# kthohr/mcmc

Measured on AMD Instinct MI355X. Metric: leapfrog-steps/sec (chains*dims*steps/s), HMC d=128 correlated Gaussian, 65536 chains, higher is better.
Workload: dtype f64

## Files before the change

mcmc_amd/csrc/logistic_dense_m_impl.hpp:

```cpp
#pragma once
#include "logistic_lds_impl.hpp"

namespace mi {
namespace {

constexpr int dense_m_matrices(int algo) { return algo == LOGIT_MALA ? 3 : 2; }

template <int NTQ, int TARGET>
size_t dense_m_doubles(uint32_t d, uint64_t C, int algo)
{
    using G = LogitGeo<NTQ>;
    const size_t nbm = (d + 15) / 16, n_wg = (C + 31) / 32;
    return (size_t)dense_m_matrices(algo) * nbm * G::XBUF_PAD + (TARGET == LOGIT_TARGET_DENSE ? 0 : n_wg * 2 * 4 * G::NSQ * 64);
}

template <int NTQ, int ALGO, int TARGET>
int launch_dense_m(LogitParams& prm, const double* X_dev, const double* y_dev, void* workspace, void* mws, hipStream_t st)
{
    using G = LogitGeo<NTQ>;
    const size_t n_wg = (prm.C + 31) / 32;
    const uint32_t nbm = (prm.d + 15) / 16;
    const size_t img = (size_t)nbm * G::XBUF_PAD;
    double* xp = static_cast<double*>(workspace);
    prm.state = xp + (size_t)prm.NB * G::XBUF_PAD;
    double* m0 = static_cast<double*>(mws);
    prm.xexch = (TARGET == LOGIT_TARGET_DENSE) ? prm.state + n_wg * 8 * LOGIT_STATE_VECS * G::NSQ * 64 : m0 + (size_t)dense_m_matrices(ALGO) * img;
    prm.Xp = xp;
    hipLaunchKernelGGL((pack_logit_lds_kernel<NTQ, TARGET == LOGIT_TARGET_DENSE>), dim3(prm.NB), dim3(256), 0, st, X_dev, y_dev, prm.d, prm.n_rows, xp);
    auto pack = [&](const double* rm, double* dst) {
        hipLaunchKernelGGL((pack_logit_lds_kernel<NTQ, true>), dim3(nbm), dim3(256), 0, st, rm, nullptr, prm.d, prm.d, dst);
    };
    prm.Lp = m0; pack(prm.L_rm, m0);
    if (ALGO == LOGIT_MALA) {
        prm.Mp = m0 + img; pack(prm.M_rm, m0 + img);
        prm.Sip = m0 + 2 * img; pack(prm.Sinv_rm, m0 + 2 * img);
    } else {
        prm.Mip = m0 + img; pack(prm.Minv_rm, m0 + img);
    }
    auto kern = logit_lds_kernel<NTQ, ALGO, TARGET, false, false, true>;
    note_kernel("logit_lds_kernel<%d, %d, %d, false, false, true>", NTQ, ALGO, TARGET);
    hipError_t e = hipFuncSetAttribute(reinterpret_cast<const void*>(kern), hipFuncAttributeMaxDynamicSharedMemorySize, (int)G::LDS_BYTES);
    if (e != hipSuccess) return (int)e;
    hipLaunchKernelGGL(kern, dim3((unsigned)n_wg), dim3(512), G::LDS_BYTES, st, prm);
    return (int)hipGetLastError();
}

template <int ALGO>
int launch_dense_m_any(LogitParams& prm, const double* X_dev, const double* y_dev, void* workspace, void* mws, hipStream_t st, int target)
{
    if (target == LOGIT_TARGET_DENSE) {
        if (prm.d <= 192) return launch_dense_m<3, ALGO, LOGIT_TARGET_DENSE>(prm, X_dev, y_dev, workspace, mws, st);
        if (prm.d <= 256) return launch_dense_m<4, ALGO, LOGIT_TARGET_DENSE>(prm, X_dev, y_dev, workspace, mws, st);
        if (prm.d <= 384) return launch_dense_m<6, ALGO, LOGIT_TARGET_DENSE>(prm, X_dev, y_dev, workspace, mws, st);
        return launch_dense_m<8, ALGO, LOGIT_TARGET_DENSE>(prm, X_dev, y_dev, workspace, mws, st);
    }
    if (prm.d <= 64) return launch_dense_m<1, ALGO, LOGIT_TARGET_LOGISTIC>(prm, X_dev, y_dev, workspace, mws, st);
    if (prm.d <= 128) return launch_dense_m<2, ALGO, LOGIT_TARGET_LOGISTIC>(prm, X_dev, y_dev, workspace, mws, st);
    if (prm.d <= 256) return launch_dense_m<4, ALGO, LOGIT_TARGET_LOGISTIC>(prm, X_dev, y_dev, workspace, mws, st);
    return launch_dense_m<8, ALGO, LOGIT_TARGET_LOGISTIC>(prm, X_dev, y_dev, workspace, mws, st);
}

}
}
```

mcmc_amd/csrc/logistic_launch.hpp:

```cpp
#pragma once

#include <hip/hip_runtime.h>
#include <stddef.h>
#include <stdint.h>

namespace mi {

struct LogitParams {
    const double* Xp;
    uint32_t d, n_rows, NB;
    uint64_t C, chain0;
    double* theta;
    double* state;
    double* draws;
    uint64_t* n_accept;
    uint64_t seed;
    uint32_t n_burnin, n_keep, n_leap;
    uint32_t draw0;
    double eps, s2, rs, cons_term, log_det;
    uint32_t* nf_flag;
    const double* m_sqrt;
    const double* m_inv;
    const double* m;
    const double* s_inv;
    const int* btype;
    const double* lb;
    const double* ub;
    double* xexch;
    double* nuts_ws;
    double* nuts_sc;
    uint32_t* nuts_next;
    uint64_t* n_leap_out;
    uint64_t* n_exec_out;
    double* step_out;
    uint32_t* depth_trace;
    double* adapt_state;
    uint32_t n_adapt, max_depth;
    double delta, eps_bar0, gamma, t0, kappa;
    const double* Minv_rm;
    const double* L_rm;
    const double* M_rm;
    const double* Sinv_rm;
    const double* Mip;
    const double* Lp;
    const double* Mp;
    const double* Sip;
    uint32_t n_pieces, piece_len;
    uint32_t* piece_q;
    uint32_t* piece_tail;
    void* split_ws;
};

enum { LOGIT_MALA = 0, LOGIT_HMC = 1, LOGIT_RWMH = 2, LOGIT_NUTS = 3 };
enum { LOGIT_TARGET_LOGISTIC = 0, LOGIT_TARGET_DENSE = 1 };

size_t logit_lds_workspace_bytes(uint32_t d, uint32_t NB, uint64_t C, int target = LOGIT_TARGET_LOGISTIC, int algo = LOGIT_HMC);
uint64_t logit_lds_nuts_workgroups(uint32_t d, uint64_t C, int target);
size_t logit_lds_nuts_split_bytes(uint64_t C, uint32_t d);
size_t logit_lds_dense_m_bytes(uint32_t d, uint64_t C, int target, int algo);
int logit_lds_launch_dense_m(int algo, LogitParams prm, const double* X_dev, const double* y_dev, void* workspace, void* mws, hipStream_t st, int target);
size_t logit_lds_nuts_dense_m_bytes(uint32_t d, uint64_t C, int target);
uint64_t logit_lds_nuts_dense_m_workgroups(uint32_t d, uint64_t C, int target);
int logit_lds_launch_nuts_dense_m(LogitParams prm, const double* X_dev, const double* y_dev, void* workspace, void* mws, hipStream_t st, int target);
int logit_lds_launch_hmc_dense_m(LogitParams prm, const double* X_dev, const double* y_dev, void* workspace, void* mws, hipStream_t st, int target);
int logit_lds_launch_mala_dense_m(LogitParams prm, const double* X_dev, const double* y_dev, void* workspace, void* mws, hipStream_t st, int target);
int logit_lds_launch(int algo, LogitParams prm, const double* X_dev, const double* y_dev, void* workspace, hipStream_t st,
                     int target = LOGIT_TARGET_LOGISTIC);

}
```

mcmc_amd/csrc/logistic_lds.hpp:

```cpp
#pragma once

#include "hmc_dense.hpp"
#include "logistic_launch.hpp"
#include "nuts_lds.hpp"
#include "lds_box.hpp"

#ifndef MI_LOGIT_ABLATE
#define MI_LOGIT_ABLATE 0
#endif
#ifndef MI_LOGIT_BATCH
#define MI_LOGIT_BATCH 8
#endif

namespace mi {


constexpr int LOGIT_STATE_VECS = 3;

template <int NTQ>
struct LogitGeo {
    static constexpr int NSQ = 4 * NTQ;
    static constexpr int DQ = 16 * NTQ;
    static constexpr int DP = 64 * NTQ;
    static constexpr int RSP = 2 * DP + 34;
    static constexpr int XBUF = 8 * RSP;
    static constexpr int CHUNKS = (XBUF * 8 + 1023) / 1024;
    static constexpr int XBUF_PAD = CHUNKS * 128;
    static_assert(CHUNKS * 128 >= XBUF + 16, "no room for the labels");
    static constexpr int EXCH = 2 * (4 * 4 * 64 + 4 * 2 * 64);
    static constexpr size_t LDS_BYTES = (size_t)(2 * XBUF_PAD + EXCH) * sizeof(double);
    __host__ __device__ static constexpr int xaddr(int row, int dim) { return (row >> 1) * RSP + (row & 1) * (DP + 16) + dim; }
};

template <int NTQ>
inline size_t logit_lds_ws_doubles(uint32_t NB, uint64_t C, int target, int algo)
{
    using G = LogitGeo<NTQ>;
    const size_t n_wg = (C + 31) / 32;
    return (size_t)NB * G::XBUF_PAD + n_wg * 8 * LOGIT_STATE_VECS * G::NSQ * 64 + (target == LOGIT_TARGET_DENSE ? n_wg * 2 * 4 * G::NSQ * 64 : 0)
           + (algo == LOGIT_NUTS ? n_wg * 8 * (lds_nuts::vec_doubles_per_wave(G::NSQ) + lds_nuts::sc_doubles_per_wave()) + 32 : 0);
}
int logit_lds_launch_nuts(LogitParams prm, const double* X_dev, const double* y_dev, void* workspace, hipStream_t st, int target);

template <int NTQ, bool TRANSPOSED>
__global__ void pack_logit_lds_kernel(const double* __restrict__ X, const double* __restrict__ y, uint32_t d, uint32_t n_rows,
                                      double* Xp)
{
    using G = LogitGeo<NTQ>;
    const uint32_t b = blockIdx.x;
    double* img = Xp + (size_t)b * G::XBUF_PAD;
    for (int i = threadIdx.x; i < G::XBUF_PAD; i += blockDim.x) img[i] = 0.0;
    __syncthreads();
    for (int i = threadIdx.x; i < 16 * G::DP; i += blockDim.x) {
        const int r = i / G::DP, j = i % G::DP;
        const uint32_t row = 16 * b + r;
        if (row < n_rows && (uint32_t)j < d) img[G::xaddr(r, j)] = TRANSPOSED ? X[(size_t)j * d + row] : X[(size_t)row * d + j];
    }
    if (!TRANSPOSED && threadIdx.x < 16) {
        const uint32_t row = 16 * b + threadIdx.x;
        img[G::XBUF + threadIdx.x] = row < n_rows ? y[row] : 0.0;
    }
}

#ifndef MI_LOGIT_NUTS_W1
#define MI_LOGIT_NUTS_W1 2
#endif
template <int NTQ, int ALGO> constexpr int logit_waves_per_simd() { return (ALGO == LOGIT_NUTS && NTQ == 1) ? MI_LOGIT_NUTS_W1 : 2; }
template <int NTQ, int ALGO, int TARGET, bool DIAGM = false, bool BOUNDS = false, bool DENSEM = false>
__global__ MI_NO_DS_MERGE __launch_bounds__(512, (logit_waves_per_simd<NTQ, ALGO>())) void logit_lds_kernel(const LogitParams prm)
{
    static_assert(!BOUNDS || (DIAGM && (ALGO == LOGIT_HMC || ALGO == LOGIT_NUTS)), "bounds: hmc and nuts, with the mass tables");
    static_assert(!DENSEM || ((ALGO == LOGIT_HMC || ALGO == LOGIT_MALA || ALGO == LOGIT_NUTS) && !DIAGM && !BOUNDS), "a dense precond_mat: hmc, mala and nuts without bounds");
    using G = LogitGeo<NTQ>;
    constexpr int NSQ = G::NSQ, DQ = G::DQ, DP = G::DP, RSP = G::RSP;
    extern __shared__ double smem[];
    double* const Xs = smem;
    double* const part_all = smem + 2 * G::XBUF_PAD;
    double* const rt_all = part_all + 2 * 4 * 4 * 64;

    const int lane = threadIdx.x & 63;
    const int w = __builtin_amdgcn_readfirstlane((int)(threadIdx.x >> 6));
    const int g = w >> 2, q = w & 3;
    const int j4 = lane >> 4;
    const uint32_t d = prm.d;
    const uint64_t C = prm.C;
    const double eps = prm.eps;
    const uint32_t NB = prm.NB;
    constexpr uint32_t ablate = MI_LOGIT_ABLATE;
    const uint64_t t0_clk = (ablate & 1024u) ? clock64() : 0, t0_wall = (ablate & 1024u) ? wall_clock64() : 0;
    const uint64_t cl = ((uint64_t)blockIdx.x * 2 + g) * 16 + (lane & 15);
    const bool live = cl < C;
    const uint64_t chain = prm.chain0 + cl;
    double* const part = part_all + g * (4 * 4 * 64);
    double* const rt = rt_all + g * (4 * 2 * 64);
    double* const ws_wave = prm.state + ((size_t)blockIdx.x * 8 + w) * ((size_t)LOGIT_STATE_VECS * NSQ * 64) + lane;
    auto st = [&](int v, int s) -> double* {
        double* b = ws_wave + ((size_t)v * NSQ + (s & ~7)) * 64;
        asm volatile("" : "+v"(b));
        return b + (s & 7) * 64;
    };
    auto dim_of = [&](int s) -> uint32_t {
        uint32_t j = (uint32_t)j4;
        asm volatile("" : "+v"(j));
        return (uint32_t)(q * DQ + 4 * s) + j;
    };

    [[maybe_unused]] auto mass_at = [&](const double* tab, int s) __attribute__((always_inline)) -> double {
        uint32_t off = (uint32_t)j4 * 8u;
        asm volatile("" : "+v"(off));
        return *reinterpret_cast<const double*>(reinterpret_cast<const char*>(tab + (q * DQ + 4 * s)) + off);
    };

    const int eta_off = G::xaddr(lane & 15, q * DQ + j4);
    const int grad_off = (j4 >> 1) * RSP + (j4 & 1) * (DP + 16) + q * DQ + (lane & 15);

    const uint32_t xs_lds = (uint32_t)(uintptr_t)(__attribute__((address_space(3))) double*)Xs;
    auto issue_block = [&](uint32_t b, int buf) __attribute__((always_inline)) {
        const double* src = prm.Xp + (size_t)b * G::XBUF_PAD + lane * 2;
        const uint32_t dst = xs_lds + (uint32_t)buf * (uint32_t)(G::XBUF_PAD * sizeof(double));
#pragma unroll
        for (int c0 = 0; c0 < G::CHUNKS; c0 += 8) {
            const int c = c0 + w;
            if (c < G::CHUNKS) {
                uint32_t m0_saved;
                asm volatile("s_mov_b32 %0, m0\n\ts_mov_b32 m0, %2\n\ts_nop 0\n\tglobal_load_lds_dwordx4 %1, off\n\ts_mov_b32 m0, %0"
                             : "=&s"(m0_saved) : "v"(src + (size_t)c * 128), "s"(dst + (uint32_t)c * 1024u) : "memory");
            }
        }
    };
    const uint32_t lane16 = (uint32_t)lane * 16u;
    auto issue_piece_of = [&](const double* img, uint32_t b, int buf, int i) __attribute__((always_inline)) {
        const int c = i * 8 + w;
        if (c < G::CHUNKS) {
            const double* src = img + (size_t)b * G::XBUF_PAD + (size_t)c * 128;
            const uint32_t dst = xs_lds + (uint32_t)buf * (uint32_t)(G::XBUF_PAD * sizeof(double)) + (uint32_t)c * 1024u;
            uint32_t m0_saved;
            asm volatile("s_mov_b32 %0, m0\n\ts_mov_b32 m0, %2\n\ts_nop 0\n\tglobal_load_lds_dwordx4 %1, %3\n\ts_mov_b32 m0, %0"
                         : "=&s"(m0_saved) : "v"(lane16), "s"(dst), "s"(src) : "memory");
        }
    };
    const double* next_img = prm.Xp;
    auto img_of_next = [&](const double* img, bool last) __attribute__((always_inline)) -> const double* {
        if constexpr (DENSEM) return last ? next_img : img; else return prm.Xp;
    };
    constexpr int NP = (G::CHUNKS + 7) / 8, NP_E = (NTQ + 1) / 2;
    static_assert(NP_E + 1 + (NTQ + 1) / 2 >= NP, "piece schedule does not cover the block");
    auto wait_loads = [&]() __attribute__((always_inline)) { asm volatile("s_waitcnt vmcnt(0)" ::: "memory"); };

    auto exchange = [&](double (&v)[2]) __attribute__((always_inline)) {
        __syncthreads();
        part[(0 * 4 + q) * 64 + lane] = v[0];
        part[(1 * 4 + q) * 64 + lane] = v[1];
        __syncthreads();
#pragma unroll
        for (int k = 0; k < 2; ++k)
            v[k] = ((part[(k * 4 + 0) * 64 + lane] + part[(k * 4 + 1) * 64 + lane]) + part[(k * 4 + 2) * 64 + lane])
                   + part[(k * 4 + 3) * 64 + lane];
    };

    auto blk_sync = [&]() __attribute__((always_inline)) { if constexpr (!(ablate & 16u)) __syncthreads(); };
    uint64_t prof[11] = {0, 0, 0, 0, 0, 0, 0, 0, 0, 0, 0};
    auto stamp = [&]() __attribute__((always_inline)) -> uint64_t { if constexpr ((ablate & 2048u) != 0) return clock64(); else return 0; };
    auto lap = [&](uint64_t& tp, int i) __attribute__((always_inline)) {
        if constexpr ((ablate & 2048u) != 0) { const uint64_t t = clock64(); prof[i] += t - tp; tp = t; }
    };
    uint32_t xbuf_next = 0;
    auto xbuf_parity = [&]() __attribute__((always_inline)) -> uint32_t {
        if constexpr (ALGO == LOGIT_NUTS) return (uint32_t)__builtin_amdgcn_readfirstlane((int)xbuf_next); else return xbuf_next;
    };
    auto evaluate_logit = [&](const double (&x)[NSQ], double (&gout)[NSQ], double& lp) __attribute__((always_inline)) {
        double4_t gacc[NTQ];
        double llq = 0.0;
#pragma unroll
        for (int t = 0; t < NTQ; ++t) gacc[t] = double4_t{0.0, 0.0, 0.0, 0.0};
        uint64_t te = stamp();
        const uint32_t xbuf0 = xbuf_parity();
        __syncthreads();
        lap(te, 8);
#pragma unroll 1
        for (uint32_t b = 0; b < NB; ++b) {
            const double* xb = Xs + ((xbuf0 + b) & 1u) * G::XBUF_PAD;
            uint64_t tp = stamp();
            const bool prefetch = !(ablate & 8u);
            const uint32_t nblk = (b + 1 < NB) ? b + 1 : 0u;
            const int nbuf = (int)((xbuf0 + b + 1) & 1u);
            const double* const nimg = img_of_next(prm.Xp, b + 1 >= NB);
            auto issue_piece = [&](uint32_t bb, int buf, int i) __attribute__((always_inline)) { issue_piece_of(nimg, bb, buf, i); };
            if (prefetch && (ablate & 4096u)) issue_block(nblk, nbuf);
            double4_t acc = double4_t{0.0, 0.0, 0.0, 0.0}, acc1 = double4_t{0.0, 0.0, 0.0, 0.0};
            {
                const double* xe = xb + eta_off;
                constexpr int H = NSQ / 2;
                double a_cur[4], a_nxt[4];
                auto frag = [&](int k, int i) -> const double* { return xe + 4 * ((i & 1) * H + 2 * k + (i >> 1)); };
#pragma unroll
                for (int i = 0; i < 4; ++i) a_cur[i] = (ablate & 32u) ? 1.0 : *frag(0, i);
#pragma unroll
                for (int k = 0; k < NSQ / 4; ++k) {
                    if (k + 1 < NSQ / 4) {
#pragma unroll
                        for (int i = 0; i < 4; ++i) a_nxt[i] = (ablate & 32u) ? 1.0 : *frag(k + 1, i);
                    }
                    __builtin_amdgcn_sched_barrier(0);
                    if ((k & 1) == 0 && k / 2 < NP_E && prefetch && !(ablate & (512u | 4096u))) issue_piece(nblk, nbuf, k / 2);
                    if constexpr (!(ablate & 2u)) {
                        acc = __builtin_amdgcn_mfma_f64_16x16x4f64(a_cur[0], x[2 * k], acc, 0, 0, 0);
                        acc1 = __builtin_amdgcn_mfma_f64_16x16x4f64(a_cur[1], x[H + 2 * k], acc1, 0, 0, 0);
                        acc = __builtin_amdgcn_mfma_f64_16x16x4f64(a_cur[2], x[2 * k + 1], acc, 0, 0, 0);
                        acc1 = __builtin_amdgcn_mfma_f64_16x16x4f64(a_cur[3], x[H + 2 * k + 1], acc1, 0, 0, 0);
                    } else {
                        acc[0] += a_cur[0] + a_cur[1] + a_cur[2] + a_cur[3];
                    }
                    __builtin_amdgcn_sched_barrier(0);
#pragma unroll
                    for (int i = 0; i < 4; ++i) a_cur[i] = a_nxt[i];
                }
                acc[0] = acc[0] + acc1[0]; acc[1] = acc[1] + acc1[1]; acc[2] = acc[2] + acc1[2]; acc[3] = acc[3] + acc1[3];
            }
            lap(tp, 0);
            part[(q * 4 + 0) * 64 + lane] = acc[0]; part[(q * 4 + 1) * 64 + lane] = acc[1];
            part[(q * 4 + 2) * 64 + lane] = acc[2]; part[(q * 4 + 3) * 64 + lane] = acc[3];
            blk_sync();
            lap(tp, 1);
            if (prefetch && (ablate & 512u)) issue_block(nblk, nbuf);
            if (prefetch && !(ablate & (512u | 4096u))) issue_piece(nblk, nbuf, NP_E);
            const double* xg = xb + grad_off;
            double g_cur[4], g_nxt[4];
#pragma unroll
            for (int sp = 0; sp < 4; ++sp) g_cur[sp] = (ablate & 32u) ? 1.0 : xg[2 * sp * RSP];
            {
                const uint32_t row = 16 * b + 4 * q + j4;
                const double yv = xb[G::XBUF + 4 * q + j4];
                const bool valid = row < prm.n_rows;
                const double eta = ((part[(0 * 4 + q) * 64 + lane] + part[(1 * 4 + q) * 64 + lane]) + part[(2 * 4 + q) * 64 + lane])
                                   + part[(3 * 4 + q) * 64 + lane];
#ifdef MI_LOGIT_ESTRIN
                double e, l1p;
                {
                    const double x = eta > 0.0 ? -eta : eta;
                    const double kf = __builtin_rint(x * INV_LN2);
                    const int k = (int)kf;
                    double r = dfma(-kf, LN2_HI, x);
                    r = dfma(-kf, LN2_LO, r);
                    const double r2 = r * r, r4 = r2 * r2, r8 = r4 * r4;
                    const double a0 = dfma(r, 1.0, 1.0), a1 = dfma(r, MI_KC(1.0 / 6.0), 0.5), a2 = dfma(r, MI_KC(1.0 / 120.0), MI_KC(1.0 / 24.0)), a3 = dfma(r, MI_KC(1.0 / 5040.0), MI_KC(1.0 / 720.0));
                    const double a4 = dfma(r, MI_KC(1.0 / 362880.0), MI_KC(1.0 / 40320.0)), a5 = dfma(r, MI_KC(1.0 / 39916800.0), MI_KC(1.0 / 3628800.0)), a6 = dfma(r, MI_KC(1.0 / 6227020800.0), MI_KC(1.0 / 479001600.0));
                    const double b0 = dfma(r2, a1, a0), b1 = dfma(r2, a3, a2), b2 = dfma(r2, a5, a4), b3 = dfma(r2, MI_KC(1.0 / 87178291200.0), a6);
                    const double d0 = dfma(r4, b1, b0), d1 = dfma(r4, b3, b2);
                    const double pe = dfma(r8, d1, d0);
                    const int k1 = k / 2, k2 = k - k1;
                    e = (x < -745.2) ? 0.0 : (pe * pow2i(k1)) * pow2i(k2);
                    double m = 1.0 + e;
                    const bool big = m > 0x1.6a09e667f3bcdp+0;
                    m = big ? m * 0.5 : m;
                    const double ef = big ? 1.0 : 0.0;
                    const double f = m - 1.0;
                    const double sq = f / (2.0 + f);
                    const double z = sq * sq, z2 = z * z, z4 = z2 * z2, z8 = z4 * z4;
                    const double c0 = dfma(z, MI_KC(1.0 / 3.0), 1.0), c1 = dfma(z, MI_KC(1.0 / 7.0), MI_KC(1.0 / 5.0)), c2 = dfma(z, MI_KC(1.0 / 11.0), MI_KC(1.0 / 9.0)), c3 = dfma(z, MI_KC(1.0 / 15.0), MI_KC(1.0 / 13.0));
                    const double c4 = dfma(z, MI_KC(1.0 / 19.0), MI_KC(1.0 / 17.0)), c5 = dfma(z, MI_KC(1.0 / 23.0), MI_KC(1.0 / 21.0));
                    const double g0 = dfma(z2, c1, c0), g1 = dfma(z2, c3, c2), g2 = dfma(z2, c5, c4);
                    const double h0 = dfma(z4, g1, g0);
                    const double pl = dfma(z8, g2, h0);
                    l1p = dfma(ef, LN2_HI, dfma(ef, LN2_LO, (2.0 * sq) * pl));
                }
#else
                const double e = (ablate & 1u) ? eta * 0.25 : det_exp(eta > 0.0 ? -eta : eta);
                const double l1p = (ablate & 1u) ? e * 0.5 : det_log(1.0 + e);
#endif
                const double sp = (eta > 0.0) ? (eta + l1p) : l1p;
                const double sg = (eta >= 0.0) ? (1.0 / (1.0 + e)) : (e / (1.0 + e));
                rt[(q * 2 + 0) * 64 + lane] = valid ? (yv - sg) : 0.0;
                rt[(q * 2 + 1) * 64 + lane] = valid ? (yv * eta - sp) : 0.0;
            }
            lap(tp, 2);
            blk_sync();
            lap(tp, 3);
            double res[4];
#pragma unroll
            for (int r = 0; r < 4; ++r) { res[r] = rt[(r * 2 + 0) * 64 + lane]; llq = llq + rt[(r * 2 + 1) * 64 + lane]; }
            {
#pragma unroll
                for (int t = 0; t < NTQ; ++t) {
                    if (t + 1 < NTQ) {
#pragma unroll
                        for (int sp = 0; sp < 4; ++sp) g_nxt[sp] = (ablate & 32u) ? 1.0 : xg[2 * sp * RSP + 16 * (t + 1)];
                    }
                    __builtin_amdgcn_sched_barrier(0);
                    if ((t & 1) == 0 && NP_E + 1 + t / 2 < NP && prefetch && !(ablate & (512u | 4096u))) issue_piece(nblk, nbuf, NP_E + 1 + t / 2);
#pragma unroll
                    for (int sp = 0; sp < 4; ++sp)
                    { if constexpr (!(ablate & 4u)) gacc[t] = __builtin_amdgcn_mfma_f64_16x16x4f64(g_cur[sp], res[sp], gacc[t], 0, 0, 0); else gacc[t][0] += g_cur[sp]; }
                    __builtin_amdgcn_sched_barrier(0);
#pragma unroll
                    for (int sp = 0; sp < 4; ++sp) g_cur[sp] = g_nxt[sp];
                }
            }
            lap(tp, 4);
            if constexpr (!(ablate & 128u)) wait_loads();
            lap(tp, 5);
            blk_sync();
            lap(tp, 6);
        }
        xbuf_next = (xbuf0 + NB) & 1u;
        te = stamp();
        llq = llq + __shfl_xor(llq, 32);
        llq = llq + __shfl_xor(llq, 16);
        double v[2];
        {
            double nrm = 0.0;
#pragma unroll
            for (int s = 0; s < NSQ; ++s) nrm = dfma(x[s], x[s], nrm);
            nrm = nrm + __shfl_xor(nrm, 32);
            nrm = nrm + __shfl_xor(nrm, 16);
            v[0] = nrm; v[1] = 0.0;
        }
        exchange(v);
#pragma unroll
        for (int t = 0; t < NTQ; ++t) {
            gout[4 * t + 0] = gacc[t][0] - x[4 * t + 0];
            gout[4 * t + 1] = gacc[t][1] - x[4 * t + 1];
            gout[4 * t + 2] = gacc[t][2] - x[4 * t + 2];
            gout[4 * t + 3] = gacc[t][3] - x[4 * t + 3];
        }
        lp = llq - 0.5 * v[0];
        lap(te, 9);
    };


    auto stream_product = [&](const double* img, uint32_t nb, const double (&x)[NSQ], double4_t (&gacc)[NTQ]) __attribute__((always_inline)) {
#pragma unroll
        for (int t = 0; t < NTQ; ++t) gacc[t] = double4_t{0.0, 0.0, 0.0, 0.0};
        const uint32_t xbuf0 = xbuf_parity();
        double* const xq_base = prm.xexch + ((size_t)blockIdx.x * 2 + g) * ((size_t)4 * NSQ * 64);
        uint32_t xq_off = (uint32_t)lane * 8u;
        asm volatile("" : "+v"(xq_off));
        auto xq_at = [&](uint32_t slot) __attribute__((always_inline)) -> double* {
            return reinterpret_cast<double*>(reinterpret_cast<char*>(xq_base) + ((size_t)slot * 512u + xq_off));
        };
#pragma unroll
        for (int s = 0; s < NSQ; ++s) *xq_at((uint32_t)(q * NSQ + s)) = x[s];
        __syncthreads();
        double r_cur[4], r_nxt[4];
#pragma unroll
        for (int sp = 0; sp < 4; ++sp) r_cur[sp] = *xq_at((uint32_t)sp);
        constexpr bool prefetch = !(ablate & 8u);
#pragma unroll 1
        for (uint32_t b = 0; b < nb; ++b) {
            const double* xb = Xs + ((xbuf0 + b) & 1u) * G::XBUF_PAD;
            const uint32_t nblk = (b + 1 < nb) ? b + 1 : 0u;
            const int nbuf = (int)((xbuf0 + b + 1) & 1u);
            const uint32_t bn = (b + 1 < nb) ? b + 1 : b;
            const double* const nimg = img_of_next(img, b + 1 >= nb);
            auto issue_piece = [&](uint32_t bb, int buf, int i) __attribute__((always_inline)) { issue_piece_of(nimg, bb, buf, i); };
#pragma unroll
            for (int sp = 0; sp < 4; ++sp) r_nxt[sp] = *xq_at(4u * bn + (uint32_t)sp);
            const double* xg = xb + grad_off;
#ifndef MI_DENSE_TT
#define MI_DENSE_TT 1
#endif
            constexpr int TT = (NTQ % MI_DENSE_TT == 0) ? MI_DENSE_TT : 1;
            double g_cur[TT][4], g_nxt[TT][4];
#pragma unroll
            for (int u = 0; u < TT; ++u)
#pragma unroll
                for (int sp = 0; sp < 4; ++sp) g_cur[u][sp] = (ablate & 32u) ? 1.0 : xg[2 * sp * RSP + 16 * u];
#pragma unroll
            for (int t = 0; t < NTQ; t += TT) {
                if (t + TT < NTQ) {
#pragma unroll
                    for (int u = 0; u < TT; ++u)
#pragma unroll
                        for (int sp = 0; sp < 4; ++sp) g_nxt[u][sp] = (ablate & 32u) ? 1.0 : xg[2 * sp * RSP + 16 * (t + TT + u)];
                }
                __builtin_amdgcn_sched_barrier(0);
#ifndef MI_DENSE_DMA_TILES
#define MI_DENSE_DMA_TILES 0
#endif
                if constexpr (prefetch) {
                    constexpr int DT = (MI_DENSE_DMA_TILES > 0 && MI_DENSE_DMA_TILES < NTQ) ? MI_DENSE_DMA_TILES : NTQ;
                    if (t < DT) {
#pragma unroll
                        for (int i = (t * NP) / DT; i < ((t + TT) * NP) / DT && i < NP; ++i) issue_piece(nblk, nbuf, i);
                    }
                }
#pragma unroll
                for (int sp = 0; sp < 4; ++sp)
#pragma unroll
                    for (int u = 0; u < TT; ++u)
                    { if constexpr (!(ablate & 4u)) gacc[t + u] = __builtin_amdgcn_mfma_f64_16x16x4f64(g_cur[u][sp], r_cur[sp], gacc[t + u], 0, 0, 0); else gacc[t + u][0] += g_cur[u][sp] * r_cur[sp]; }
                __builtin_amdgcn_sched_barrier(0);
#pragma unroll
                for (int u = 0; u < TT; ++u)
#pragma unroll
                    for (int sp = 0; sp < 4; ++sp) g_cur[u][sp] = g_nxt[u][sp];
            }
            if constexpr (!(ablate & 128u)) wait_loads();
#pragma unroll
            for (int sp = 0; sp < 4; ++sp) r_cur[sp] = r_nxt[sp];
            blk_sync();
        }
        xbuf_next = (xbuf0 + nb) & 1u;
    };
    auto evaluate_dense = [&](const double (&x)[NSQ], double (&gout)[NSQ], double& lp) __attribute__((always_inline)) {
        double4_t gacc[NTQ];
        stream_product(prm.Xp, NB, x, gacc);
        double v[2];
        {
            double a = 0.0;
#pragma unroll
            for (int s = 0; s < NSQ; ++s) a = dfma(x[s], gacc[s >> 2][s & 3], a);
            a = a + __shfl_xor(a, 32);
            a = a + __shfl_xor(a, 16);
            v[0] = a; v[1] = 0.0;
        }
        exchange(v);
#pragma unroll
        for (int s = 0; s < NSQ; ++s) gout[s] = -gacc[s >> 2][s & 3];
        lp = -0.5 * v[0];
    };
    auto evaluate = [&](const double (&x)[NSQ], double (&gout)[NSQ], double& lp) __attribute__((always_inline)) {
        if constexpr (TARGET == LOGIT_TARGET_DENSE) evaluate_dense(x, gout, lp); else evaluate_logit(x, gout, lp);
    };

    double bp[NSQ], gp[NSQ];
#pragma unroll
    for (int s = 0; s < NSQ; ++s) {
        const uint32_t dim = dim_of(s);
        const double v = prm.theta[(size_t)(dim < d ? dim : 0u) * C + (live ? cl : C - 1)];
        bp[s] = (dim < d) ? v : 0.0;
    }
    [[maybe_unused]] LdsBox<NTQ> box;
    [[maybe_unused]] double* const lj_rel = part + (3 * 4) * 64 + 32;
    if constexpr (BOUNDS && ALGO == LOGIT_HMC) {
        box.init(prm.btype, prm.lb, prm.ub, d, q, lane);
#pragma unroll
        for (int s = 0; s < NSQ; ++s) bp[s] = (dim_of(s) < d) ? box.enter(bp[s], s) : 0.0;
    }
    auto evaluate_at = [&](double (&t)[NSQ], double (&gout)[NSQ], double& lp) __attribute__((always_inline)) {
        if constexpr (BOUNDS) {
#pragma unroll
            for (int s = 0; s < NSQ; ++s) *st(2, s) = t[s];
            box.x_inplace(t);
            evaluate(t, gout, lp);
#pragma unroll
            for (int s = 0; s < NSQ; ++s) t[s] = *st(2, s);
        } else evaluate(t, gout, lp);
    };
    issue_block(0, 0);
    wait_loads();
    if constexpr (ALGO == LOGIT_NUTS) {
        struct DenseMOps {
            decltype(stream_product)& sp; decltype(issue_piece_of)& ip; decltype(wait_loads)& wl; decltype(xbuf_parity)& xp;
            const double*& nimg; uint32_t nbm;
            __device__ __forceinline__ void product(const double* img, const double* next, const double (&x)[NSQ], double4_t (&acc)[NTQ]) const { nimg = next; sp(img, nbm, x, acc); }
            __device__ __forceinline__ void next(const double* img) const { nimg = img; }
            __device__ __forceinline__ void reload0(const double* img) const
            {
                const int buf = (int)xp();
#pragma unroll
                for (int i = 0; i < NP; ++i) ip(img, 0u, buf, i);
                wl();
                __syncthreads();
            }
        };
        DenseMOps dm{stream_product, issue_piece_of, wait_loads, xbuf_parity, next_img, (d + 15u) / 16u};
        nuts_lds_body<NTQ, DIAGM, BOUNDS, DENSEM>(prm, evaluate, part_all, dm);
        return;
    }
    double first_lp;
    if constexpr (DENSEM) next_img = (ALGO == LOGIT_MALA) ? prm.Mp : prm.Lp;
    evaluate_at(bp, gp, first_lp);
    if constexpr (BOUNDS) first_lp = first_lp + box.log_jacobian(bp, lj_rel, [&]() { __syncthreads(); });
#pragma unroll
    for (int s = 0; s < NSQ; ++s) { *st(0, s) = bp[s]; *st(1, s) = gp[s]; }
    uint64_t n_acc = 0;
    const uint32_t n_total = prm.n_burnin + prm.n_keep;
    constexpr uint64_t NF_BIT = 1ull << 63;

    constexpr int SB0 = (MI_LOGIT_BATCH == 0) ? 2 : ((NSQ < MI_LOGIT_BATCH) ? NSQ : MI_LOGIT_BATCH);
    constexpr int SB = (NSQ % SB0 == 0) ? SB0 : 4;
#ifndef MI_LOGIT_NT_DRAWS
#define MI_LOGIT_NT_DRAWS 0
#endif
    auto put_row = [&](double* p_, double v_) __attribute__((always_inline)) {
#if MI_LOGIT_NT_DRAWS
        __builtin_nontemporal_store(v_, p_);
#else
        *p_ = v_;
#endif
    };
    auto keep_draw = [&](uint32_t draw, bool accept) __attribute__((always_inline)) {
        if (draw >= prm.n_burnin) {
            n_acc += accept ? 1u : 0u;
            if (prm.draws != nullptr) {
                double* out = prm.draws + (size_t)(draw - prm.n_burnin) * d * C + cl;
                if (__any(!accept)) {
#pragma unroll
                    for (int s0 = 0; s0 < NSQ; s0 += SB) {
                        double old[SB];
#pragma unroll
                        for (int i = 0; i < SB; ++i) old[i] = *st(0, s0 + i);
#pragma unroll
                        for (int i = 0; i < SB; ++i) {
                            const uint32_t dim = dim_of(s0 + i);
                            double v = accept ? bp[s0 + i] : old[i];
                            if constexpr (BOUNDS) v = box.leave(v, s0 + i);
                            if (live && dim < d) put_row(out + (size_t)dim * C, v);
                        }
                    }
                } else {
#pragma unroll
                    for (int s = 0; s < NSQ; ++s) {
                        const uint32_t dim = dim_of(s);
                        double v = bp[s];
                        if constexpr (BOUNDS) v = box.leave(v, s);
                        if (live && dim < d) put_row(out + (size_t)dim * C, v);
                    }
                }
            }
        }
    };

    if constexpr (ALGO == LOGIT_MALA && DENSEM) {
        const uint32_t NBM = (d + 15u) / 16u;
        const double s2 = prm.s2;
        double prev_LP = first_lp, prop_LP;
        double4_t acc[NTQ];
        next_img = prm.Lp;
        stream_product(prm.Mp, NBM, gp, acc);
#pragma unroll
        for (int s = 0; s < NSQ; ++s) *st(2, s) = acc[s >> 2][s & 3];
        auto quad = [&]() __attribute__((always_inline)) -> double {
            double a = 0.0;
#pragma unroll
            for (int s = 0; s < NSQ; ++s) a = dfma(gp[s], acc[s >> 2][s & 3], a);
            a = a + __shfl_xor(a, 32);
            a = a + __shfl_xor(a, 16);
            return a;
        };
#pragma unroll 1
        for (uint32_t draw = 0; draw < n_total; ++draw) {
#pragma unroll
            for (int m = 0; m < NSQ / 2; ++m) {
                double z0, z1;
                const uint32_t slot = (uint32_t)(q * DQ / 2 + 4 * m + j4);
                rng_normal_pair(prm.seed, chain, draw + prm.draw0, slot, STREAM_NORMAL, z0, z1);
                bp[2 * m] = (dim_of(2 * m) < d) ? z0 : 0.0;
                bp[2 * m + 1] = (dim_of(2 * m + 1) < d) ? z1 : 0.0;
                __builtin_amdgcn_sched_barrier(0);
            }
            next_img = prm.Xp;
            stream_product(prm.Lp, NBM, bp, acc);
#pragma unroll
// ... 333 lines not shown
```

mcmc_amd/csrc/logistic_lds_impl.hpp:

```cpp
#pragma once
#include "logistic_lds.hpp"
#include "launch_common.hpp"

namespace mi {
namespace {

template <int NTQ>
size_t ws_doubles(uint32_t NB, uint64_t C, int target, int algo)
{
    return logit_lds_ws_doubles<NTQ>(NB, C, target, algo);
}

template <int NTQ, int ALGO, int TARGET, bool DIAGM = false, bool BOUNDS = false>
int launch(LogitParams& prm, const double* X_dev, const double* y_dev, void* workspace, hipStream_t st)
{
    if constexpr ((ALGO == LOGIT_HMC || ALGO == LOGIT_MALA) && !DIAGM) {
        if (prm.m_sqrt != nullptr) return launch<NTQ, ALGO, TARGET, true>(prm, X_dev, y_dev, workspace, st);
    }
    using G = LogitGeo<NTQ>;
    const size_t n_wg = (prm.C + 31) / 32;
    double* xp = static_cast<double*>(workspace);
    prm.state = xp + (size_t)prm.NB * G::XBUF_PAD;
    prm.xexch = (TARGET == LOGIT_TARGET_DENSE) ? prm.state + n_wg * 8 * LOGIT_STATE_VECS * G::NSQ * 64 : nullptr;
    prm.Xp = xp;
    hipLaunchKernelGGL((pack_logit_lds_kernel<NTQ, TARGET == LOGIT_TARGET_DENSE>), dim3(prm.NB), dim3(256), 0, st, X_dev, y_dev, prm.d, prm.n_rows, xp);
    auto kern = logit_lds_kernel<NTQ, ALGO, TARGET, DIAGM, BOUNDS>;
    if (BOUNDS) note_kernel("logit_lds_kernel<%d, %d, %d, true, true>", NTQ, ALGO, TARGET);
    else note_kernel("logit_lds_kernel<%d, %d, %d, %s>", NTQ, ALGO, TARGET, DIAGM ? "true" : "false");
    hipError_t e = hipFuncSetAttribute(reinterpret_cast<const void*>(kern), hipFuncAttributeMaxDynamicSharedMemorySize, (int)G::LDS_BYTES);
    if (e != hipSuccess) return (int)e;
    hipLaunchKernelGGL(kern, dim3((unsigned)n_wg), dim3(512), G::LDS_BYTES, st, prm);
    return (int)hipGetLastError();
}

template <int ALGO, bool BOUNDS = false>
int launch_any(LogitParams& prm, const double* X_dev, const double* y_dev, void* workspace, hipStream_t st, int target)
{
    if (target == LOGIT_TARGET_DENSE) {
        if (prm.d <= 192) return launch<3, ALGO, LOGIT_TARGET_DENSE, BOUNDS, BOUNDS>(prm, X_dev, y_dev, workspace, st);
        if (prm.d <= 256) return launch<4, ALGO, LOGIT_TARGET_DENSE, BOUNDS, BOUNDS>(prm, X_dev, y_dev, workspace, st);
        if (prm.d <= 384) return launch<6, ALGO, LOGIT_TARGET_DENSE, BOUNDS, BOUNDS>(prm, X_dev, y_dev, workspace, st);
        return launch<8, ALGO, LOGIT_TARGET_DENSE, BOUNDS, BOUNDS>(prm, X_dev, y_dev, workspace, st);
    }
    if (prm.d <= 64) return launch<1, ALGO, LOGIT_TARGET_LOGISTIC, BOUNDS, BOUNDS>(prm, X_dev, y_dev, workspace, st);
    if (prm.d <= 128) return launch<2, ALGO, LOGIT_TARGET_LOGISTIC, BOUNDS, BOUNDS>(prm, X_dev, y_dev, workspace, st);
    if (prm.d <= 256) return launch<4, ALGO, LOGIT_TARGET_LOGISTIC, BOUNDS, BOUNDS>(prm, X_dev, y_dev, workspace, st);
    return launch<8, ALGO, LOGIT_TARGET_LOGISTIC, BOUNDS, BOUNDS>(prm, X_dev, y_dev, workspace, st);
}

}
int logit_lds_launch_hmc_box(LogitParams prm, const double* X_dev, const double* y_dev, void* workspace, hipStream_t st, int target);
}
```

mcmc_amd/csrc/logistic_nuts_dense_m.hip:

```cpp
#define MI_KC_MODE 2
#define MI_RNG_NOINLINE 1
#include "logistic_lds.hpp"
#include "launch_common.hpp"
#include "lds_nuts_pieces.hpp"

namespace mi {
namespace {

template <int NTQ, int TARGET>
uint64_t grid_dm(uint64_t C)
{
    using G = LogitGeo<NTQ>;
    int dev = 0, n_cu = 256, per_cu = 1;
    (void)hipGetDevice(&dev);
    (void)hipDeviceGetAttribute(&n_cu, hipDeviceAttributeMultiprocessorCount, dev);
    if (n_cu <= 0) n_cu = 256;
    auto kern = logit_lds_kernel<NTQ, LOGIT_NUTS, TARGET, false, false, true>;
    (void)hipFuncSetAttribute(reinterpret_cast<const void*>(kern), hipFuncAttributeMaxDynamicSharedMemorySize, (int)G::LDS_BYTES);
    if (hipOccupancyMaxActiveBlocksPerMultiprocessor(&per_cu, reinterpret_cast<const void*>(kern), 512, G::LDS_BYTES) != hipSuccess || per_cu < 1) per_cu = 1;
    const uint64_t need = (C + 31) / 32, cap = (uint64_t)n_cu * (uint64_t)per_cu;
    return cap_grid(need < cap ? need : cap);
}

template <int NTQ, int TARGET>
size_t nuts_dense_m_doubles(uint32_t d, uint64_t C)
{
    using G = LogitGeo<NTQ>;
    const size_t nbm = (d + 15) / 16, n_wg = (size_t)grid_dm<NTQ, TARGET>(C);
    return 2 * nbm * G::XBUF_PAD + (TARGET == LOGIT_TARGET_DENSE ? 0 : n_wg * 2 * 4 * G::NSQ * 64);
}

template <int NTQ, int TARGET>
int launch_nuts_dense_m(LogitParams& prm, const double* X_dev, const double* y_dev, void* workspace, void* mws, hipStream_t st)
{
    using G = LogitGeo<NTQ>;
    const size_t n_wg = (size_t)grid_dm<NTQ, TARGET>(prm.C);
    const uint32_t nbm = (prm.d + 15) / 16;
    const size_t img = (size_t)nbm * G::XBUF_PAD;
    double* xp = static_cast<double*>(workspace);
    prm.state = xp + (size_t)prm.NB * G::XBUF_PAD;
    double* nxt = prm.state + n_wg * 8 * LOGIT_STATE_VECS * G::NSQ * 64;
    double* m0 = static_cast<double*>(mws);
    if (TARGET == LOGIT_TARGET_DENSE) { prm.xexch = nxt; nxt += n_wg * 2 * 4 * G::NSQ * 64; }
    else prm.xexch = m0 + 2 * img;
    prm.nuts_ws = nxt;
    prm.nuts_sc = nxt + n_wg * 8 * lds_nuts::vec_doubles_per_wave(G::NSQ);
    prm.nuts_next = reinterpret_cast<uint32_t*>(prm.nuts_sc + n_wg * 8 * lds_nuts::sc_doubles_per_wave());
    prm.Xp = xp;
    hipError_t e = hipMemsetAsync(prm.nuts_next, 0, 64, st);
    if (e != hipSuccess) return (int)e;
    double* theta_backup = nullptr;
    if (int ep = lds_nuts_setup_pieces<NTQ>(prm, n_wg, st, &theta_backup)) return ep;
    hipLaunchKernelGGL((pack_logit_lds_kernel<NTQ, TARGET == LOGIT_TARGET_DENSE>), dim3(prm.NB), dim3(256), 0, st, X_dev, y_dev, prm.d, prm.n_rows, xp);
    auto pack = [&](const double* rm, double* dst) {
        hipLaunchKernelGGL((pack_logit_lds_kernel<NTQ, true>), dim3(nbm), dim3(256), 0, st, rm, nullptr, prm.d, prm.d, dst);
    };
    prm.Lp = m0; pack(prm.L_rm, m0);
    prm.Mip = m0 + img; pack(prm.Minv_rm, m0 + img);
    auto kern = logit_lds_kernel<NTQ, LOGIT_NUTS, TARGET, false, false, true>;
    note_kernel("logit_lds_kernel<%d, nuts, %d, false, false, true>", NTQ, TARGET);
    e = hipFuncSetAttribute(reinterpret_cast<const void*>(kern), hipFuncAttributeMaxDynamicSharedMemorySize, (int)G::LDS_BYTES);
    if (e != hipSuccess) return (int)e;
    hipLaunchKernelGGL(kern, dim3((unsigned)n_wg), dim3(512), G::LDS_BYTES, st, prm);
    return lds_nuts_restore_flagged(prm, theta_backup, st);
}

}

uint64_t logit_lds_nuts_dense_m_workgroups(uint32_t d, uint64_t C, int target)
{
    if (target == LOGIT_TARGET_DENSE)
        return d <= 192 ? grid_dm<3, LOGIT_TARGET_DENSE>(C) : d <= 256 ? grid_dm<4, LOGIT_TARGET_DENSE>(C)
             : d <= 384 ? grid_dm<6, LOGIT_TARGET_DENSE>(C) : grid_dm<8, LOGIT_TARGET_DENSE>(C);
    return d <= 64 ? grid_dm<1, LOGIT_TARGET_LOGISTIC>(C) : d <= 128 ? grid_dm<2, LOGIT_TARGET_LOGISTIC>(C)
         : d <= 256 ? grid_dm<4, LOGIT_TARGET_LOGISTIC>(C) : grid_dm<8, LOGIT_TARGET_LOGISTIC>(C);
}

size_t logit_lds_nuts_dense_m_bytes(uint32_t d, uint64_t C, int target)
{
    const size_t n = (target == LOGIT_TARGET_DENSE)
                         ? ((d <= 192) ? nuts_dense_m_doubles<3, LOGIT_TARGET_DENSE>(d, C) : (d <= 256) ? nuts_dense_m_doubles<4, LOGIT_TARGET_DENSE>(d, C)
                            : (d <= 384) ? nuts_dense_m_doubles<6, LOGIT_TARGET_DENSE>(d, C) : nuts_dense_m_doubles<8, LOGIT_TARGET_DENSE>(d, C))
                   : (d <= 64) ? nuts_dense_m_doubles<1, LOGIT_TARGET_LOGISTIC>(d, C) : (d <= 128) ? nuts_dense_m_doubles<2, LOGIT_TARGET_LOGISTIC>(d, C)
                   : (d <= 256) ? nuts_dense_m_doubles<4, LOGIT_TARGET_LOGISTIC>(d, C) : nuts_dense_m_doubles<8, LOGIT_TARGET_LOGISTIC>(d, C);
    return n * sizeof(double);
}

int logit_lds_launch_nuts_dense_m(LogitParams prm, const double* X_dev, const double* y_dev, void* workspace, void* mws, hipStream_t st, int target)
{
    if (target == LOGIT_TARGET_DENSE) {
        if (prm.d <= 192) return launch_nuts_dense_m<3, LOGIT_TARGET_DENSE>(prm, X_dev, y_dev, workspace, mws, st);
        if (prm.d <= 256) return launch_nuts_dense_m<4, LOGIT_TARGET_DENSE>(prm, X_dev, y_dev, workspace, mws, st);
        if (prm.d <= 384) return launch_nuts_dense_m<6, LOGIT_TARGET_DENSE>(prm, X_dev, y_dev, workspace, mws, st);
        return launch_nuts_dense_m<8, LOGIT_TARGET_DENSE>(prm, X_dev, y_dev, workspace, mws, st);
    }
    if (prm.d <= 64) return launch_nuts_dense_m<1, LOGIT_TARGET_LOGISTIC>(prm, X_dev, y_dev, workspace, mws, st);
    if (prm.d <= 128) return launch_nuts_dense_m<2, LOGIT_TARGET_LOGISTIC>(prm, X_dev, y_dev, workspace, mws, st);
    if (prm.d <= 256) return launch_nuts_dense_m<4, LOGIT_TARGET_LOGISTIC>(prm, X_dev, y_dev, workspace, mws, st);
    return launch_nuts_dense_m<8, LOGIT_TARGET_LOGISTIC>(prm, X_dev, y_dev, workspace, mws, st);
}

}
```

mcmc_amd/csrc/logistic_nuts_impl.hpp:

```cpp
#pragma once
#include "logistic_lds.hpp"
#include "launch_common.hpp"
#include "lds_nuts_pieces.hpp"

namespace mi {
namespace {

template <int NTQ, int TARGET>
uint64_t grid_of(uint64_t C)
{
    using G = LogitGeo<NTQ>;
    int dev = 0, n_cu = 256, per_cu = 1;
    (void)hipGetDevice(&dev);
    (void)hipDeviceGetAttribute(&n_cu, hipDeviceAttributeMultiprocessorCount, dev);
    if (n_cu <= 0) n_cu = 256;
    auto kern = logit_lds_kernel<NTQ, LOGIT_NUTS, TARGET, false>;
    (void)hipFuncSetAttribute(reinterpret_cast<const void*>(kern), hipFuncAttributeMaxDynamicSharedMemorySize, (int)G::LDS_BYTES);
    if (hipOccupancyMaxActiveBlocksPerMultiprocessor(&per_cu, reinterpret_cast<const void*>(kern), 512, G::LDS_BYTES) != hipSuccess || per_cu < 1) per_cu = 1;
    const uint64_t need = (C + 31) / 32, cap = (uint64_t)n_cu * (uint64_t)per_cu;
    return cap_grid(need < cap ? need : cap);
}

template <int NTQ, int TARGET, bool DIAGM = false, bool BOUNDS = false>
int launch_nuts(LogitParams& prm, const double* X_dev, const double* y_dev, void* workspace, hipStream_t st)
{
    using G = LogitGeo<NTQ>;
    const size_t n_wg = (size_t)grid_of<NTQ, TARGET>(prm.C);
    double* xp = static_cast<double*>(workspace);
    prm.state = xp + (size_t)prm.NB * G::XBUF_PAD;
    double* nxt = prm.state + n_wg * 8 * LOGIT_STATE_VECS * G::NSQ * 64;
    prm.xexch = nullptr;
    if (TARGET == LOGIT_TARGET_DENSE) { prm.xexch = nxt; nxt += n_wg * 2 * 4 * G::NSQ * 64; }
    prm.nuts_ws = nxt;
    prm.nuts_sc = nxt + n_wg * 8 * lds_nuts::vec_doubles_per_wave(G::NSQ);
    prm.nuts_next = reinterpret_cast<uint32_t*>(prm.nuts_sc + n_wg * 8 * lds_nuts::sc_doubles_per_wave());
    prm.Xp = xp;
    hipError_t e = hipMemsetAsync(prm.nuts_next, 0, 64, st);
    if (e != hipSuccess) return (int)e;
    double* theta_backup = nullptr;
    if (int ep = lds_nuts_setup_pieces<NTQ>(prm, n_wg, st, &theta_backup)) return ep;
    hipLaunchKernelGGL((pack_logit_lds_kernel<NTQ, TARGET == LOGIT_TARGET_DENSE>), dim3(prm.NB), dim3(256), 0, st, X_dev, y_dev, prm.d, prm.n_rows, xp);
    auto kern = logit_lds_kernel<NTQ, LOGIT_NUTS, TARGET, DIAGM, BOUNDS>;
    if (BOUNDS) note_kernel("logit_lds_kernel<%d, nuts, %d, true, true>", NTQ, TARGET);
    else note_kernel("logit_lds_kernel<%d, nuts, %d, %s>", NTQ, TARGET, DIAGM ? "true" : "false");
    e = hipFuncSetAttribute(reinterpret_cast<const void*>(kern), hipFuncAttributeMaxDynamicSharedMemorySize, (int)G::LDS_BYTES);
    if (e != hipSuccess) return (int)e;
    hipLaunchKernelGGL(kern, dim3((unsigned)n_wg), dim3(512), G::LDS_BYTES, st, prm);
    if ((e = hipGetLastError()) != hipSuccess) return (int)e;
    return lds_nuts_restore_flagged(prm, theta_backup, st);
}

template <bool DIAGM, bool BOUNDS>
int dispatch_nuts(LogitParams& prm, const double* X_dev, const double* y_dev, void* workspace, hipStream_t st, int target)
{
    if (target == LOGIT_TARGET_DENSE) {
        if (prm.d <= 192) return launch_nuts<3, LOGIT_TARGET_DENSE, DIAGM, BOUNDS>(prm, X_dev, y_dev, workspace, st);
        if (prm.d <= 256) return launch_nuts<4, LOGIT_TARGET_DENSE, DIAGM, BOUNDS>(prm, X_dev, y_dev, workspace, st);
        if (prm.d <= 384) return launch_nuts<6, LOGIT_TARGET_DENSE, DIAGM, BOUNDS>(prm, X_dev, y_dev, workspace, st);
        return launch_nuts<8, LOGIT_TARGET_DENSE, DIAGM, BOUNDS>(prm, X_dev, y_dev, workspace, st);
    }
    if (prm.d <= 64) return launch_nuts<1, LOGIT_TARGET_LOGISTIC, DIAGM, BOUNDS>(prm, X_dev, y_dev, workspace, st);
    if (prm.d <= 128) return launch_nuts<2, LOGIT_TARGET_LOGISTIC, DIAGM, BOUNDS>(prm, X_dev, y_dev, workspace, st);
    if (prm.d <= 256) return launch_nuts<4, LOGIT_TARGET_LOGISTIC, DIAGM, BOUNDS>(prm, X_dev, y_dev, workspace, st);
    return launch_nuts<8, LOGIT_TARGET_LOGISTIC, DIAGM, BOUNDS>(prm, X_dev, y_dev, workspace, st);
}

}
int logit_lds_launch_nuts_box(LogitParams prm, const double* X_dev, const double* y_dev, void* workspace, hipStream_t st, int target);
}
```

Baseline: 266.8 billion.

## Exchange position blocks through an LDS ring instead of a global scratch buffer

The dense-target gradient previously wrote each wave's full position vector to a per-workgroup global scratch area (xexch) and read 4-double slices back each block iteration. It now publishes only the next-needed block into a 3-slot ring carved from the existing LDS partials area, rotating slots per iteration. This removes global memory round-trips and the workspace allocation, but adds per-iteration LDS writes and relies on the existing block sync for ordering. Timing stamps (lap) are inserted too.

```diff
diff --git a/mcmc_amd/csrc/logistic_dense_m_impl.hpp b/mcmc_amd/csrc/logistic_dense_m_impl.hpp
--- a/mcmc_amd/csrc/logistic_dense_m_impl.hpp
+++ b/mcmc_amd/csrc/logistic_dense_m_impl.hpp
@@ -10,8 +10,9 @@
 size_t dense_m_doubles(uint32_t d, uint64_t C, int algo)
 {
     using G = LogitGeo<NTQ>;
-    const size_t nbm = (d + 15) / 16, n_wg = (C + 31) / 32;
-    return (size_t)dense_m_matrices(algo) * nbm * G::XBUF_PAD + (TARGET == LOGIT_TARGET_DENSE ? 0 : n_wg * 2 * 4 * G::NSQ * 64);
+    const size_t nbm = (d + 15) / 16;
+    (void)C;
+    return (size_t)dense_m_matrices(algo) * nbm * G::XBUF_PAD;
 }
 
 template <int NTQ, int ALGO, int TARGET>
@@ -24,7 +25,6 @@
     double* xp = static_cast<double*>(workspace);
     prm.state = xp + (size_t)prm.NB * G::XBUF_PAD;
     double* m0 = static_cast<double*>(mws);
-    prm.xexch = (TARGET == LOGIT_TARGET_DENSE) ? prm.state + n_wg * 8 * LOGIT_STATE_VECS * G::NSQ * 64 : m0 + (size_t)dense_m_matrices(ALGO) * img;
     prm.Xp = xp;
     hipLaunchKernelGGL((pack_logit_lds_kernel<NTQ, TARGET == LOGIT_TARGET_DENSE>), dim3(prm.NB), dim3(256), 0, st, X_dev, y_dev, prm.d, prm.n_rows, xp);
     auto pack = [&](const double* rm, double* dst) {
diff --git a/mcmc_amd/csrc/logistic_launch.hpp b/mcmc_amd/csrc/logistic_launch.hpp
--- a/mcmc_amd/csrc/logistic_launch.hpp
+++ b/mcmc_amd/csrc/logistic_launch.hpp
@@ -26,7 +26,6 @@
     const int* btype;
     const double* lb;
     const double* ub;
-    double* xexch;
     double* nuts_ws;
     double* nuts_sc;
     uint32_t* nuts_next;
diff --git a/mcmc_amd/csrc/logistic_lds.hpp b/mcmc_amd/csrc/logistic_lds.hpp
--- a/mcmc_amd/csrc/logistic_lds.hpp
+++ b/mcmc_amd/csrc/logistic_lds.hpp
@@ -37,7 +37,8 @@
 {
     using G = LogitGeo<NTQ>;
     const size_t n_wg = (C + 31) / 32;
-    return (size_t)NB * G::XBUF_PAD + n_wg * 8 * LOGIT_STATE_VECS * G::NSQ * 64 + (target == LOGIT_TARGET_DENSE ? n_wg * 2 * 4 * G::NSQ * 64 : 0)
+    (void)target;
+    return (size_t)NB * G::XBUF_PAD + n_wg * 8 * LOGIT_STATE_VECS * G::NSQ * 64
            + (algo == LOGIT_NUTS ? n_wg * 8 * (lds_nuts::vec_doubles_per_wave(G::NSQ) + lds_nuts::sc_doubles_per_wave()) + 32 : 0);
 }
 int logit_lds_launch_nuts(LogitParams prm, const double* X_dev, const double* y_dev, void* workspace, hipStream_t st, int target);
@@ -332,29 +333,52 @@
 #pragma unroll
         for (int t = 0; t < NTQ; ++t) gacc[t] = double4_t{0.0, 0.0, 0.0, 0.0};
         const uint32_t xbuf0 = xbuf_parity();
-        double* const xq_base = prm.xexch + ((size_t)blockIdx.x * 2 + g) * ((size_t)4 * NSQ * 64);
-        uint32_t xq_off = (uint32_t)lane * 8u;
-        asm volatile("" : "+v"(xq_off));
-        auto xq_at = [&](uint32_t slot) __attribute__((always_inline)) -> double* {
-            return reinterpret_cast<double*>(reinterpret_cast<char*>(xq_base) + ((size_t)slot * 512u + xq_off));
+        auto ring_at = [&](uint32_t slot) __attribute__((always_inline)) -> double* {
+            return part_all + (slot == 2u ? (uint32_t)(g * (4 * 4 * 64) + 2 * 4 * 64) : (uint32_t)(2 * 4 * 4 * 64 + g * (4 * 64)) + slot * (uint32_t)(2 * 4 * 64)) + lane;
         };
-#pragma unroll
-        for (int s = 0; s < NSQ; ++s) *xq_at((uint32_t)(q * NSQ + s)) = x[s];
+        auto publish = [&](uint32_t bb, uint32_t slot) __attribute__((always_inline)) {
+            const uint32_t rel = bb - (uint32_t)(q * NTQ);
+            double* const dst = ring_at(slot);
+#pragma unroll
+            for (int t = 0; t < NTQ; ++t) {
+                if (rel == (uint32_t)t) {
+#pragma unroll
+                    for (int sp = 0; sp < 4; ++sp) { asm volatile("" :: "v"(x[4 * t + sp])); dst[sp * 64] = x[4 * t + sp]; }
+                }
+            }
+        };
+#pragma unroll
+        for (int s = 0; s < NSQ; ++s) asm volatile("" : "+v"(const_cast<double&>(x[s])));
+        uint64_t ts = stamp();
+        publish(0u, 0u);
+        publish(1u, 1u);
+        lap(ts, 0);
         __syncthreads();
+        lap(ts, 1);
         double r_cur[4], r_nxt[4];
-#pragma unroll
-        for (int sp = 0; sp < 4; ++sp) r_cur[sp] = *xq_at((uint32_t)sp);
+        {
+            const double* const r0 = ring_at(0u);
+#pragma unroll
+            for (int sp = 0; sp < 4; ++sp) r_cur[sp] = r0[sp * 64];
+        }
+        if constexpr ((ablate & 2048u) != 0) asm volatile("s_waitcnt vmcnt(0) lgkmcnt(0)" ::: "memory");
+        lap(ts, 2);
         constexpr bool prefetch = !(ablate & 8u);
+        uint32_t s0 = 0u, s1 = 1u, s2 = 2u;
 #pragma unroll 1
         for (uint32_t b = 0; b < nb; ++b) {
             const double* xb = Xs + ((xbuf0 + b) & 1u) * G::XBUF_PAD;
             const uint32_t nblk = (b + 1 < nb) ? b + 1 : 0u;
             const int nbuf = (int)((xbuf0 + b + 1) & 1u);
-            const uint32_t bn = (b + 1 < nb) ? b + 1 : b;
             const double* const nimg = img_of_next(img, b + 1 >= nb);
             auto issue_piece = [&](uint32_t bb, int buf, int i) __attribute__((always_inline)) { issue_piece_of(nimg, bb, buf, i); };
-#pragma unroll
-            for (int sp = 0; sp < 4; ++sp) r_nxt[sp] = *xq_at(4u * bn + (uint32_t)sp);
+            {
+                const double* const rn = ring_at((b + 1 < nb) ? s1 : s0);
+#pragma unroll
+                for (int sp = 0; sp < 4; ++sp) r_nxt[sp] = rn[sp * 64];
+            }
+            if (b + 2 < nb) publish(b + 2u, s2);
+            { const uint32_t t_ = s0; s0 = s1; s1 = s2; s2 = t_; }
             const double* xg = xb + grad_off;
 #ifndef MI_DENSE_TT
 #define MI_DENSE_TT 1
@@ -400,6 +424,8 @@
             for (int sp = 0; sp < 4; ++sp) r_cur[sp] = r_nxt[sp];
             blk_sync();
         }
+        lap(ts, 3);
+        if constexpr ((ablate & 2048u) != 0) prof[4] += 1;
         xbuf_next = (xbuf0 + nb) & 1u;
     };
     auto evaluate_dense = [&](const double (&x)[NSQ], double (&gout)[NSQ], double& lp) __attribute__((always_inline)) {
diff --git a/mcmc_amd/csrc/logistic_lds_impl.hpp b/mcmc_amd/csrc/logistic_lds_impl.hpp
--- a/mcmc_amd/csrc/logistic_lds_impl.hpp
+++ b/mcmc_amd/csrc/logistic_lds_impl.hpp
@@ -21,7 +21,6 @@
     const size_t n_wg = (prm.C + 31) / 32;
     double* xp = static_cast<double*>(workspace);
     prm.state = xp + (size_t)prm.NB * G::XBUF_PAD;
-    prm.xexch = (TARGET == LOGIT_TARGET_DENSE) ? prm.state + n_wg * 8 * LOGIT_STATE_VECS * G::NSQ * 64 : nullptr;
     prm.Xp = xp;
     hipLaunchKernelGGL((pack_logit_lds_kernel<NTQ, TARGET == LOGIT_TARGET_DENSE>), dim3(prm.NB), dim3(256), 0, st, X_dev, y_dev, prm.d, prm.n_rows, xp);
     auto kern = logit_lds_kernel<NTQ, ALGO, TARGET, DIAGM, BOUNDS>;
diff --git a/mcmc_amd/csrc/logistic_nuts_dense_m.hip b/mcmc_amd/csrc/logistic_nuts_dense_m.hip
--- a/mcmc_amd/csrc/logistic_nuts_dense_m.hip
+++ b/mcmc_amd/csrc/logistic_nuts_dense_m.hip
@@ -26,8 +26,9 @@
 size_t nuts_dense_m_doubles(uint32_t d, uint64_t C)
 {
     using G = LogitGeo<NTQ>;
-    const size_t nbm = (d + 15) / 16, n_wg = (size_t)grid_dm<NTQ, TARGET>(C);
-    return 2 * nbm * G::XBUF_PAD + (TARGET == LOGIT_TARGET_DENSE ? 0 : n_wg * 2 * 4 * G::NSQ * 64);
+    const size_t nbm = (d + 15) / 16;
+    (void)C;
+    return 2 * nbm * G::XBUF_PAD;
 }
 
 template <int NTQ, int TARGET>
@@ -41,8 +42,6 @@
     prm.state = xp + (size_t)prm.NB * G::XBUF_PAD;
     double* nxt = prm.state + n_wg * 8 * LOGIT_STATE_VECS * G::NSQ * 64;
     double* m0 = static_cast<double*>(mws);
-    if (TARGET == LOGIT_TARGET_DENSE) { prm.xexch = nxt; nxt += n_wg * 2 * 4 * G::NSQ * 64; }
-    else prm.xexch = m0 + 2 * img;
     prm.nuts_ws = nxt;
     prm.nuts_sc = nxt + n_wg * 8 * lds_nuts::vec_doubles_per_wave(G::NSQ);
     prm.nuts_next = reinterpret_cast<uint32_t*>(prm.nuts_sc + n_wg * 8 * lds_nuts::sc_doubles_per_wave());
diff --git a/mcmc_amd/csrc/logistic_nuts_impl.hpp b/mcmc_amd/csrc/logistic_nuts_impl.hpp
--- a/mcmc_amd/csrc/logistic_nuts_impl.hpp
+++ b/mcmc_amd/csrc/logistic_nuts_impl.hpp
@@ -29,8 +29,6 @@
     double* xp = static_cast<double*>(workspace);
     prm.state = xp + (size_t)prm.NB * G::XBUF_PAD;
     double* nxt = prm.state + n_wg * 8 * LOGIT_STATE_VECS * G::NSQ * 64;
-    prm.xexch = nullptr;
-    if (TARGET == LOGIT_TARGET_DENSE) { prm.xexch = nxt; nxt += n_wg * 2 * 4 * G::NSQ * 64; }
     prm.nuts_ws = nxt;
     prm.nuts_sc = nxt + n_wg * 8 * lds_nuts::vec_doubles_per_wave(G::NSQ);
     prm.nuts_next = reinterpret_cast<uint32_t*>(prm.nuts_sc + n_wg * 8 * lds_nuts::sc_doubles_per_wave());
```

Result: no change. 266.8 billion, median of 4 (+0.0%).
